# finleygou/GS-MARL

Measured on NVIDIA B200. Metric: agent-steps/sec (graph obs+reward+cost) at 1/2/4/8 B200; % HBM roofline, higher is better.
Workload: dtype f32

## Files before the change

gs_marl_b200/csrc/gsm_kernels.cuh:

```cuda
#pragma once
#include <cuda_runtime.h>
#include <math.h>
#include <stdint.h>

#include "../../include/gsmarl_b200.h"
#include "gsm_host.h"

namespace gsm {

constexpr int kThreads = 128;
__host__ __device__ constexpr unsigned low_mask(int n) { return n >= 32 ? 0xffffffffu : ((1u << (n & 31)) - 1u); }

template <typename T>
struct KParams {
  int64_t n_envs, env_offset;
  int N, L, E, K, W;
  int scenario, action_mode, n_actions, episode_length;
  int share_reward, cost_obstacles, own_goal_always;
  int envs_per_warp;
  T dt, one_minus_damp, cf, km, km_inv, Rs, w_dist, w_goal, goal_tol, poly_r;
  T discrete_u[GSM_MAX_DISCRETE][2];
  const T* size;
  const uint8_t* eflag;
  const T* mass;
  const T* accel;
  const T* max_speed;
  const T* slot_table;
  T* agent_state;
  T* lm_pos;
  int32_t* t;
  const uint8_t* mask;
  int64_t mask_stride;
  int auto_reset;
  uint64_t seed;
  int32_t* episode;
  double ext[4];
  const void* actions;
  T* obs; int32_t* nbr_idx; T* nbr_feat; int32_t* nbr_cnt; uint32_t* adj;
  T* reward; T* cost; uint8_t* done; int32_t* assign;
};

struct SmemLayout {
  size_t off_size, off_agc, off_ag, off_lm, off_new, off_rew, off_slot, off_cmat, off_asg,
      off_stage, off_flag, stage_stride, stage_feat, total;
};
__host__ __device__ inline SmemLayout make_layout(int rb, int N, int L, int E, int K, int epb,
                                                  int groups, int lsa) {
  SmemLayout s;
  size_t o = 0;
  auto take = [&](size_t bytes) { size_t r = o; o += ((bytes + 15) / 16) * 16; return r; };
  s.off_size = take((size_t)E * rb);
  s.off_agc = take((size_t)N * 3 * rb);
  s.off_ag = take((size_t)epb * N * 4 * rb);
  s.off_lm = take((size_t)epb * L * 2 * rb);
  s.off_new = take((size_t)epb * N * 4 * rb);
  s.off_rew = take((size_t)epb * N * rb);
  s.off_slot = take(lsa ? (size_t)epb * N * 2 * rb : 0);
  s.off_cmat = take(lsa ? (size_t)epb * N * N * rb : 0);
  s.off_asg = take((size_t)epb * N * 4);
  s.stage_feat = (((size_t)K * 4 + 15) / 16) * 16;
  s.stage_stride = s.stage_feat + (((size_t)K * GSM_NBR_FEAT_DIM * rb + 15) / 16) * 16;
  s.off_stage = take((size_t)groups * s.stage_stride);
  s.off_flag = take((size_t)E);
  s.total = o;
  return s;
}

__device__ __forceinline__ float r_sqrt(float x) { return sqrtf(x); }
__device__ __forceinline__ double r_sqrt(double x) { return sqrt(x); }
__device__ __forceinline__ float r_exp(float x) { return expf(x); }
__device__ __forceinline__ double r_exp(double x) { return exp(x); }
__device__ __forceinline__ float r_log1p(float x) { return log1pf(x); }
__device__ __forceinline__ double r_log1p(double x) { return log1p(x); }

template <typename T>
__device__ __forceinline__ T softplus(T x) {
  if (x > (T)0) return x + r_log1p(r_exp(-x));
  return r_log1p(r_exp(x));
}

__device__ __forceinline__ float shfl(unsigned m, float v, int src) { return __shfl_sync(m, v, src); }
__device__ __forceinline__ double shfl(unsigned m, double v, int src) { return __shfl_sync(m, v, src); }
__device__ __forceinline__ int shfl(unsigned m, int v, int src) { return __shfl_sync(m, v, src); }

__device__ __forceinline__ float mask_min(unsigned m, float v) {
  unsigned b = __float_as_uint(v);
  unsigned key = (b & 0x80000000u) ? ~b : (b | 0x80000000u);
  unsigned r = __reduce_min_sync(m, key);
  return __uint_as_float((r & 0x80000000u) ? (r & 0x7fffffffu) : ~r);
}
__device__ __forceinline__ double mask_min(unsigned m, double v) {
  unsigned long long b = (unsigned long long)__double_as_longlong(v);
  unsigned long long key = (b >> 63) ? ~b : (b | 0x8000000000000000ull);
  unsigned hi = (unsigned)(key >> 32), lo = (unsigned)key;
  unsigned mhi = __reduce_min_sync(m, hi);
  unsigned mlo = __reduce_min_sync(m, hi == mhi ? lo : 0xffffffffu);
  unsigned long long r = ((unsigned long long)mhi << 32) | mlo;
  r = (r >> 63) ? (r & 0x7fffffffffffffffull) : ~r;
  return __longlong_as_double((long long)r);
}

template <typename T> __device__ __forceinline__ T r_inf();
template <> __device__ __forceinline__ float r_inf<float>() { return __int_as_float(0x7f800000); }
template <> __device__ __forceinline__ double r_inf<double>() {
  return __longlong_as_double(0x7ff0000000000000ll);
}

__device__ __forceinline__ void philox4x32_10(uint32_t c0, uint32_t c1, uint32_t c2, uint32_t c3,
                                              uint32_t k0, uint32_t k1, uint32_t out[4]);
__device__ __forceinline__ double u53(uint32_t hi, uint32_t lo);
static __device__ __noinline__ void spawn_draw_f64(uint64_t g, int ep, int e, uint64_t seed, double ext,
                                            double* x, double* y) {
  uint32_t r[4];
  philox4x32_10((uint32_t)g, (uint32_t)(g >> 32), (uint32_t)ep, (uint32_t)e, (uint32_t)seed,
                (uint32_t)(seed >> 32), r);
  *x = __dadd_rn(-ext, __dmul_rn(2.0 * ext, u53(r[0], r[1])));
  *y = __dadd_rn(-ext, __dmul_rn(2.0 * ext, u53(r[2], r[3])));
}
template <typename T>
__device__ __forceinline__ void spawn_draw(uint64_t g, int ep, int e, uint64_t seed, double ext, T& x, T& y) {
  double dx, dy;
  spawn_draw_f64(g, ep, e, seed, ext, &dx, &dy);
  x = (T)dx; y = (T)dy;
}

template <typename T> struct Prec;
template <> struct Prec<float> { static constexpr bool kCut = true; };
template <> struct Prec<double> { static constexpr bool kCut = false; };
constexpr float kFarCut = 20.0f;

template <int P>
__device__ __forceinline__ void group_copy(void* gdst, const void* ssrc, int bytes, int sub) {
  const uintptr_t ga = (uintptr_t)gdst;
  if (((ga | (uintptr_t)bytes) & 15) == 0) {
    for (int k = sub; k < (bytes >> 4); k += P) ((int4*)gdst)[k] = ((const int4*)ssrc)[k];
  } else if (((ga | (uintptr_t)bytes) & 7) == 0) {
    for (int k = sub; k < (bytes >> 3); k += P) ((int2*)gdst)[k] = ((const int2*)ssrc)[k];
  } else {
    for (int k = sub; k < (bytes >> 2); k += P) ((int*)gdst)[k] = ((const int*)ssrc)[k];
  }
}

template <typename T>
__device__ int lsa_lanes(const T* __restrict__ C, int n, int col, unsigned gm, int base) {
  const T INF = r_inf<T>();
  T u_m = 0, v_m = 0;
  int col4row_m = -1, row4col_m = -1, path_m = -1;
  const bool is_col = col < n;
  for (int cur = 0; cur < n; cur++) {
    T minval = 0, spc = INF;
    int i = cur, nrem = n, sink = -1;
    int pos = n - 1 - col;
    bool inrem = is_col, sr_m = false, sc_m = false;
    for (int iter = 0; iter < n && sink == -1; iter++) {
      if (col == i) sr_m = true;
      const T u_i = shfl(gm, u_m, base + i);
      if (inrem) {
        const T r = minval + C[i * n + col] - u_i - v_m;
        if (r < spc) { path_m = i; spc = r; }
      }
      const T lowest = mask_min(gm, inrem ? spc : INF);
      if (lowest == INF) return -1;
      const bool cand = inrem && spc == lowest;
      const bool ucand = cand && row4col_m == -1;
      const unsigned bu = __ballot_sync(gm, ucand);
      int selpos;
      if (bu) selpos = __reduce_max_sync(gm, ucand ? pos : -1);
      else selpos = __reduce_min_sync(gm, cand ? pos : 0x3fffffff);
      const bool sel = inrem && pos == selpos;
      const int jl = __ffs(__ballot_sync(gm, sel)) - 1;
      minval = lowest;
      const int r4c = shfl(gm, row4col_m, jl);
      if (r4c == -1) sink = jl - base; else i = r4c;
      if (sel) { sc_m = true; inrem = false; }
      nrem--;
      if (inrem && pos == nrem) pos = selpos;
    }
    const T spc_row = shfl(gm, spc, base + (col4row_m >= 0 ? col4row_m : 0));
    if (is_col) {
      if (col == cur) u_m += minval;
      else if (sr_m) u_m += minval - spc_row;
    }
    if (sc_m) v_m -= minval - spc;
    if (sink < 0) return -1;
    int j = sink;
    for (int iter = 0; iter < n; iter++) {
      const int a = shfl(gm, path_m, base + j);
      if (col == j) row4col_m = a;
      const int tprev = shfl(gm, col4row_m, base + a);
      if (col == a) col4row_m = j;
      j = tprev;
      if (a == cur) break;
    }
  }
  return col4row_m;
}

template <typename T, int N>
__device__ __forceinline__ int lsa_seg(const T* __restrict__ C, int off, int base, bool live) {
  constexpr unsigned FULL = 0xffffffffu;
  const T INF = r_inf<T>();
  const bool is_col = live && off < N;
  T u_m = 0, v_m = 0;
  int col4row_m = -1, row4col_m = -1, path_m = -1;
  for (int cur = 0; cur < N; cur++) {
    T minval = 0, spc = INF;
    int i = cur, nrem = N, sink = live ? -1 : 0;
    int rem = N - 1 - off;
    bool inrem = is_col, sr_m = false, sc_m = false;
    for (int iter = 0; iter < N && __any_sync(FULL, sink == -1); iter++) {
      const bool run = sink == -1;
      if (run && off == i) sr_m = true;
      const T u_i = shfl(FULL, u_m, base + i);
      if (run && inrem) {
        const T r = minval + C[i * N + off] - u_i - v_m;
        if (r < spc) { path_m = i; spc = r; }
      }
      const T mine = inrem ? spc : INF;
      T lowest = INF;
#pragma unroll
      for (int k = 0; k < N; k++) {
        const T o = shfl(FULL, mine, base + k);
        lowest = o < lowest ? o : lowest;
      }
      const int rc = off < N ? rem : 0;
      const T spc_of = shfl(FULL, spc, base + rc);
      const int r4c_of = shfl(FULL, row4col_m, base + rc);
      const bool cand = is_col && off < nrem && spc_of == lowest;
      const bool ucand = cand && r4c_of == -1;
      const unsigned bc = (__ballot_sync(FULL, cand) >> base) & low_mask(N);
      const unsigned bu = (__ballot_sync(FULL, ucand) >> base) & low_mask(N);
      const int it_sel = bu ? (31 - __clz(bu)) : (bc ? __ffs(bc) - 1 : 0);
      const int j = shfl(FULL, rem, base + it_sel);
      const int r4c_j = shfl(FULL, row4col_m, base + j);
      const int last = shfl(FULL, rem, base + nrem - 1);
      if (run) {
        minval = lowest;
        if (r4c_j == -1) sink = j; else i = r4c_j;
        if (off == j) { sc_m = true; inrem = false; }
        if (off == it_sel) rem = last;
        nrem--;
      }
    }
    const T spc_row = shfl(FULL, spc, base + (col4row_m >= 0 ? col4row_m : 0));
    if (is_col) {
      if (off == cur) u_m += minval;
      else if (sr_m) u_m += minval - spc_row;
    }
    if (sc_m) v_m -= minval - spc;
    int j = sink;
    bool going = live && sink >= 0;
    for (int iter = 0; iter < N && __any_sync(FULL, going); iter++) {
      const int a = shfl(FULL, path_m, base + j);
      const int tprev = shfl(FULL, col4row_m, base + a);
      if (going) {
        if (off == j) row4col_m = a;
        if (off == a) col4row_m = j;
        j = tprev;
        if (a == cur) going = false;
      }
    }
  }
  return col4row_m;
}

template <typename T, int P, bool CTA_ENV, bool PHYS>
__global__ void __launch_bounds__(kThreads) env_kernel(const __grid_constant__ KParams<T> p) {
  extern __shared__ __align__(16) unsigned char smem[];
  const int N = p.N, L = p.L, E = p.E, K = p.K, W = p.W;
  const bool lsa = p.scenario != GSM_SCN_NAVIGATION;
  const int EPB = CTA_ENV ? 1 : p.envs_per_warp * (kThreads / 32);
  const SmemLayout lay = make_layout((int)sizeof(T), N, L, E, K, EPB, kThreads / P, lsa ? 1 : 0);
  T* s_size = (T*)(smem + lay.off_size);
  T* s_agc = (T*)(smem + lay.off_agc);
  T* s_ag = (T*)(smem + lay.off_ag);
// ... 370 lines not shown
```

gs_marl_b200/csrc/gsm_kernels_wide.cuh:

```cuda
#pragma once
#include "gsm_kernels_spec.cuh"
#include "gsm_bulk.cuh"

namespace gsm {

constexpr int kWideThreads = 128;
__host__ __device__ constexpr int wide_pow2(int v) { int p = 1; while (p < v) p <<= 1; return p; }

template <typename T, int N, int E>
struct WideConsts {
  T size[E];
  T mass[N], mass_inv[N], accel[N], maxsp[N];
  int32_t eflag[E];
};

#ifndef GSM_WIDE_BLOCKS
#define GSM_WIDE_BLOCKS 7
#endif
template <typename T> struct WideMinBlocks { static constexpr int value = sizeof(T) == 4 ? GSM_WIDE_BLOCKS : 1; };

__device__ __forceinline__ float softplus1(float x) {
  float y, l;
  asm("ex2.approx.ftz.f32 %0, %1;" : "=f"(y) : "f"(-fabsf(x) * 1.4426950408889634f));
  asm("lg2.approx.ftz.f32 %0, %1;" : "=f"(l) : "f"(1.0f + y));
  return fmaxf(x, 0.f) + 0.6931471805599453f * l;
}
__device__ __forceinline__ double softplus1(double x) { return fmax(x, 0.0) + r_log1p(r_exp(-fabs(x))); }

__device__ __forceinline__ int keep(int v) { return __shfl_sync(0xffffffffu, v, threadIdx.x & 31); }
__device__ __forceinline__ unsigned keep(unsigned v) { return __shfl_sync(0xffffffffu, v, threadIdx.x & 31); }
__device__ __forceinline__ float keep(float v) { return __shfl_sync(0xffffffffu, v, threadIdx.x & 31); }
__device__ __forceinline__ double keep(double v) { return __shfl_sync(0xffffffffu, v, threadIdx.x & 31); }

__device__ __forceinline__ void sts(unsigned a, unsigned v) { asm volatile("st.shared.u32 [%0], %1;" :: "r"(a), "r"(v) : "memory"); }
__device__ __forceinline__ void sts(unsigned a, int v) { asm volatile("st.shared.u32 [%0], %1;" :: "r"(a), "r"(v) : "memory"); }
__device__ __forceinline__ void sts(unsigned a, float v) { asm volatile("st.shared.f32 [%0], %1;" :: "r"(a), "f"(v) : "memory"); }
__device__ __forceinline__ void sts(unsigned a, double v) { asm volatile("st.shared.f64 [%0], %1;" :: "r"(a), "d"(v) : "memory"); }
__device__ __forceinline__ void sts2(unsigned a, float x, float y) { asm volatile("st.shared.v2.f32 [%0], {%1, %2};" :: "r"(a), "f"(x), "f"(y) : "memory"); }
__device__ __forceinline__ void sts2(unsigned a, double x, double y) { asm volatile("st.shared.v2.f64 [%0], {%1, %2};" :: "r"(a), "d"(x), "d"(y) : "memory"); }
__device__ __forceinline__ void sts4(unsigned a, float x, float y, float z, float w) {
  asm volatile("st.shared.v4.f32 [%0], {%1, %2, %3, %4};" :: "r"(a), "f"(x), "f"(y), "f"(z), "f"(w) : "memory");
}
__device__ __forceinline__ void sts4(unsigned a, double x, double y, double z, double w) { sts2(a, x, y); sts2(a + 16, z, w); }
__device__ __forceinline__ void lds4(unsigned a, float& x, float& y, float& z, float& w) {
  asm volatile("ld.shared.v4.f32 {%0, %1, %2, %3}, [%4];" : "=f"(x), "=f"(y), "=f"(z), "=f"(w) : "r"(a) : "memory");
}
__device__ __forceinline__ void lds4(unsigned a, double& x, double& y, double& z, double& w) {
  asm volatile("ld.shared.v2.f64 {%0, %1}, [%2];" : "=d"(x), "=d"(y) : "r"(a) : "memory");
  asm volatile("ld.shared.v2.f64 {%0, %1}, [%2];" : "=d"(z), "=d"(w) : "r"(a + 16) : "memory");
}
__device__ __forceinline__ float4 lds16(unsigned a) {
  float4 v; asm volatile("ld.shared.v4.f32 {%0, %1, %2, %3}, [%4];" : "=f"(v.x), "=f"(v.y), "=f"(v.z), "=f"(v.w) : "r"(a) : "memory"); return v;
}

template <typename T>
__device__ __forceinline__ T shfl_xor(T v, int m) { return __shfl_xor_sync(0xffffffffu, v, m); }

template <typename T> struct __align__(16) WideEnt { T x, y, vx, vy; };

struct WideSmem {
  unsigned feat, idx, obs, cnt, adj, cost, rew, asg, buf;
  unsigned ent, warp;
};
__host__ __device__ constexpr WideSmem wide_smem_layout(int rb, int N, int E, int K, int EPW) {
  WideSmem w{};
  unsigned o = 0;
  w.feat = o; o += (unsigned)(EPW * N * K * GSM_NBR_FEAT_DIM * rb);
  w.idx = o; o += ((unsigned)(EPW * N * K * 4) + 15u) & ~15u;
  w.obs = o; o += (unsigned)(EPW * N * GSM_OBS_DIM * rb);
  w.cnt = o; o += (unsigned)(EPW * N * 4);
  w.adj = o; o += (unsigned)(EPW * N * 4);
  w.cost = o; o += (unsigned)(EPW * N * rb);
  w.rew = o; o += (unsigned)(EPW * N * rb);
  w.asg = o; o += (unsigned)(EPW * N * 4);
  w.buf = (o + 15u) & ~15u;
  w.ent = 2 * w.buf;
  w.warp = w.ent + (unsigned)(EPW * E * 4 * rb);
  return w;
}
__host__ __device__ constexpr size_t wide_smem_bytes(int rb, int N, int E, int K, int EPW) {
  return (size_t)(kWideThreads / 32) * wide_smem_layout(rb, N, E, K, EPW).warp;
}

template <typename T, int N, int L, int MODE, int KT>
__global__ void __launch_bounds__(kWideThreads, WideMinBlocks<T>::value)
env_wide_kernel(const __grid_constant__ KParams<T> p, const int n_steps,
                const __grid_constant__ StepStrides ss,
                const __grid_constant__ WideConsts<T, N, N + L> wc,
                const __grid_constant__ WideSmem lay_rt) {
  constexpr int E = N + L, M = E - 1, GW = wide_pow2(M), EPW = 32 / GW;
  constexpr bool OBS = MODE == 1;
  constexpr unsigned FULL = 0xffffffffu;
  constexpr int RB = (int)sizeof(T);
  constexpr int RS4 = EPW * N * 4, RST = EPW * N * RB;
  constexpr int PS = (RS4 % 16 == 0 && RST % 16 == 0) ? 16 : 8;
  constexpr int PC4 = RS4 / PS, PCT = RST / PS, NPIECE = 3 * PC4 + 2 * PCT;
  constexpr bool ROLE_OK = NPIECE <= 32;
  static_assert(GW <= 32 && E <= 32, "an env must fit in one warp, adjacency in one word");
  static_assert(L >= N && 2 * N <= GW + 1 && N >= 3, "goal i is landmark i, held by lane N-1+i; lanes 0..2 stage scalars");
  static_assert(RS4 % 8 == 0 && RST % 8 == 0, "per-warp scalar blocks leave in 8- or 16-byte pieces");
  static_assert(EPW * N * M * 4 / 16 <= 64 && EPW * N * GSM_OBS_DIM * RB / 16 <= 64, "idx / obs blocks leave in <= 2 passes");
  typedef Arith<T> A;
  typedef WideEnt<T> Ent;
  typedef float4 V;
  extern __shared__ __align__(128) unsigned char wsm[];
  const int K = KT > 0 ? KT : p.K;
  const WideSmem lay = KT > 0 ? wide_smem_layout((int)sizeof(T), N, N + L, KT > 0 ? KT : 1, 32 / wide_pow2(N + L - 1)) : lay_rt;
  const int lane = keep((int)(threadIdx.x & 31)), warp = threadIdx.x >> 5;
  const int grp = lane / GW, j = lane % GW, shift = grp * GW;
  const int env_w0 = keep((int)(((int64_t)blockIdx.x * (kWideThreads / 32) + warp) * EPW));
  bool active = env_w0 + grp < p.n_envs;
  if (OBS && p.mask != nullptr && active) active = p.mask[(int64_t)(env_w0 + grp) * p.mask_stride] != 0;
  const int env = active ? env_w0 + grp : 0;
  const bool has = M == GW ? true : j < M;
  const bool own = j < N;
  const int ja = own ? j : 0;
  const unsigned act_bits = __ballot_sync(FULL, active);
  const bool bulk = ROLE_OK && act_bits == FULL && ((EPW * N * K * 4) & 15) == 0 &&
      ((((uintptr_t)p.obs | (uintptr_t)p.nbr_idx | (uintptr_t)p.nbr_feat | (uintptr_t)p.nbr_cnt | (uintptr_t)p.adj |
         (uintptr_t)p.assign | (uintptr_t)p.reward | (uintptr_t)p.cost | (uintptr_t)ss.obs | (uintptr_t)ss.nbr_idx |
         (uintptr_t)ss.nbr_feat | (uintptr_t)ss.nbr_cnt | (uintptr_t)ss.adj | (uintptr_t)ss.assign |
         (uintptr_t)ss.reward | (uintptr_t)ss.cost) & 15) == 0);

  constexpr unsigned ES = (unsigned)sizeof(Ent);
  const unsigned sa_w = keep(smem_u32(wsm) + (unsigned)warp * lay.warp);
  const unsigned sa_ent = keep(smem_u32(wsm) + (unsigned)warp * lay.warp + lay.ent + (unsigned)(grp * E) * ES);

  const int e_hi = has ? j + 1 : 0;
  const int fl_o = wc.eflag[e_hi];
  const T size_o = keep(wc.size[e_hi]), type_o = keep((T)(fl_o >> 1));
  const unsigned lfl = keep((unsigned)((has && (wc.eflag[0] & 1) && (fl_o & 1)) ? 1u : 0u) |
                            ((has && (e_hi < N || (p.cost_obstacles && (fl_o >> 1) == GSM_ENT_OBSTACLE))) ? 2u : 0u) |
                            (((has && p.own_goal_always && j >= N - 1 && j < 2 * N - 1) ? (unsigned)(j - (N - 1) + 1) : 0u) << 8));
  const bool cpair = lfl & 1u, colc = lfl & 2u;
  const int goal_i = (int)(lfl >> 8) - 1;

  T mx, my, mvx, mvy;
  {
    const T* a = p.agent_state + ((int64_t)env * N + ja) * 4;
    mx = a[0]; my = a[1]; mvx = a[2]; mvy = a[3];
  }
  if (own) sts4(sa_ent + (unsigned)j * ES, mx, my, mvx, mvy);
  if (has && j + 1 >= N) {
    const T* l = p.lm_pos + ((int64_t)env * L + (j + 1 - N)) * 2;
    sts4(sa_ent + (unsigned)(j + 1) * ES, l[0], l[1], (T)0, (T)0);
  }
  int t_now = p.t[env];
  const bool auto_reset = MODE == 2 && p.auto_reset != 0;
  const T accel_m = keep(wc.accel[ja]), mass_m = keep(wc.mass[ja]), massinv_m = keep(wc.mass_inv[ja]), maxsp_m = keep(wc.maxsp[ja]);

  const unsigned char* b_act = (const unsigned char*)p.actions;
  unsigned char* b_obs = (unsigned char*)p.obs;
  unsigned char* b_idx = (unsigned char*)p.nbr_idx;
  unsigned char* b_feat = (unsigned char*)p.nbr_feat;
  unsigned char* b_done = (unsigned char*)p.done;
  const unsigned wrow0 = (unsigned)env_w0 * N;
  unsigned char* c_role = nullptr;
  int64_t role_stride = ss.nbr_cnt;
  {
    const int q = lane;
    if (q < PC4) c_role = (unsigned char*)p.nbr_cnt + wrow0 * 4u + q * PS;
    else if (q < 2 * PC4) { c_role = (unsigned char*)p.adj + wrow0 * 4u + (q - PC4) * PS; if (RB != 4) role_stride = ss.adj; }
    else if (q < 2 * PC4 + PCT) { c_role = (unsigned char*)p.cost + wrow0 * (unsigned)RB + (q - 2 * PC4) * PS; if (RB != 4) role_stride = ss.cost; }
    else if (q < 2 * PC4 + 2 * PCT) { c_role = (unsigned char*)p.reward + wrow0 * (unsigned)RB + (q - 2 * PC4 - PCT) * PS; if (RB != 4) role_stride = ss.reward; }
    else if (q < NPIECE) { c_role = (unsigned char*)p.assign + wrow0 * 4u + (q - 2 * PC4 - 2 * PCT) * PS; if (RB != 4) role_stride = ss.assign; }
  }
  const bool role_on = lane < NPIECE && (!OBS || lane < 2 * PC4 || lane >= 2 * PC4 + 2 * PCT);
  if (own) {
    sts(sa_w + lay.asg + (unsigned)(grp * N + j) * 4u, j);
    sts(sa_w + lay.buf + lay.asg + (unsigned)(grp * N + j) * 4u, j);
  }

  const bool discrete = p.action_mode == GSM_ACT_DISCRETE;
  const unsigned act_off = keep(discrete ? ((unsigned)env * N + ja) * 4u : ((unsigned)env * N + ja) * 2u * (unsigned)RB);
  const unsigned n_idx = (lay.obs - lay.idx) / 16, n_obs = (lay.cnt - lay.obs) / 16;
  const unsigned off_idx = keep(wrow0 * (unsigned)(K * 4) + (unsigned)lane * 16u), off_obs = keep(wrow0 * (unsigned)(GSM_OBS_DIM * RB) + (unsigned)lane * 16u);
  const unsigned off_done = keep((unsigned)env * N + (unsigned)ja);
  int act_next = 0;
  T actx_next = 0, acty_next = 0;
  if (!OBS) {
    if (discrete) act_next = *(const int32_t*)(b_act + act_off);
    else { actx_next = ((const T*)(b_act + act_off))[0]; acty_next = ((const T*)(b_act + act_off))[1]; }
  }
  __syncwarp();

  T fox = 0, foy = 0;
  bool pro = !OBS;
  int step = 0;
  unsigned sb = sa_w;
  int sb_delta = (int)lay.buf;
  const unsigned o_feat = keep((unsigned)(grp * N * K) * (unsigned)(GSM_NBR_FEAT_DIM * RB));
  const unsigned o_idx = keep(lay.idx + (unsigned)(grp * N * K) * 4u);
  const unsigned o_sc = keep(lay.cnt + (unsigned)(j < 3 ? j : 0) * (unsigned)RS4 + (unsigned)(grp * N) * 4u);
  const unsigned o_obs = keep(lay.obs + (unsigned)grp * (unsigned)(N * GSM_OBS_DIM * RB));
  while (step < n_steps) {
   for (;;) {
    if (!OBS && !pro) {
      T ux = actx_next, uy = acty_next;
      if (discrete) {
        const int a = act_next;
        ux = 0; uy = 0;
        if (a >= 0 && a < p.n_actions) { ux = p.discrete_u[a][0]; uy = p.discrete_u[a][1]; }
      }
      if (step + 1 < n_steps) b_act += ss.actions;
      if (discrete) act_next = *(const int32_t*)(b_act + act_off);
      else { actx_next = ((const T*)(b_act + act_off))[0]; acty_next = ((const T*)(b_act + act_off))[1]; }
      const T fx = accel_m * ux + fox, fy = accel_m * uy + foy;
      T nvx = mvx * p.one_minus_damp, nvy = mvy * p.one_minus_damp;
      nvx = nvx + A::div_const(fx, mass_m, massinv_m) * p.dt;
      nvy = nvy + A::div_const(fy, mass_m, massinv_m) * p.dt;
      if (maxsp_m > (T)0) {
        const T sp = A::sqrt(nvx * nvx + nvy * nvy);
        if (sp > maxsp_m) { nvx = A::div(nvx, sp) * maxsp_m; nvy = A::div(nvy, sp) * maxsp_m; }
      }
      mvx = nvx; mvy = nvy;
      mx = mx + nvx * p.dt; my = my + nvy * p.dt;
      t_now += 1;
      if (own) sts4(sa_ent + (unsigned)j * ES, mx, my, mvx, mvy);
      __syncwarp();
    }
    const bool st_on = !pro;
    const unsigned a_feat = sb + o_feat, a_idx = sb + o_idx, a_sc = sb + o_sc, sobs = sb + o_obs;
    if (st_on && bulk && lane == 0) bulk_wait_read<1>();

    T fcx[N], fcy[N];
    T gxs = 0, gys = 0, gd = 0;
    bool anyc = false;
#pragma unroll
    for (int i = 0; i < N; i++) {
      const int e = e_hi - (j < i ? 1 : 0);
      Ent si, so;
      lds4(sa_ent + (unsigned)i * ES, si.x, si.y, si.vx, si.vy);
      lds4(sa_ent + (unsigned)e * ES, so.x, so.y, so.vx, so.vy);
      const T dx = so.x - si.x, dy = so.y - si.y;
      const T dist = A::sqrt(dx * dx + dy * dy);
      const T dmin = wc.size[i] + size_o;
      const bool nb = (has && dist < p.Rs) || goal_i == i;
      const bool col = colc && dist < dmin;
      const unsigned bits = (__ballot_sync(FULL, nb) >> shift) & low_mask(GW);
      const unsigned cbits = (__ballot_sync(FULL, col) >> shift) & low_mask(GW);
      int cnt = __popc(bits);
      const int rank = __popc(bits & low_mask(j));
      const int pos = nb ? rank : cnt + (j - rank);
      if (has && pos < K && st_on) {
        sts(a_idx + (unsigned)pos * 4u + (unsigned)(i * K * 4), nb ? e : -1);
        const unsigned f = a_feat + (unsigned)pos * (unsigned)(GSM_NBR_FEAT_DIM * RB) + (unsigned)(i * K * GSM_NBR_FEAT_DIM * RB);
        const T z = (T)0;
        if (nb) { sts2(f, dx, dy); sts2(f + 2 * RB, so.vx - si.vx, so.vy - si.vy); sts2(f + 4 * RB, dist, type_o); }
        else { sts2(f, z, z); sts2(f + 2 * RB, z, z); sts2(f + 4 * RB, z, z); }
      }
      if (cnt > K) cnt = K;
      if (st_on && j < 3) {
        const unsigned ebits = (bits & low_mask(i)) | ((bits & ~low_mask(i)) << 1);
        const unsigned ao = (unsigned)(grp * N + i);
        if (RB == 4) {
          const unsigned v = j == 0 ? (unsigned)cnt : (j == 1 ? ebits : __float_as_uint((float)__popc(cbits)));
          if (!OBS || j < 2) sts(a_sc + (unsigned)(i * 4), v);
        } else {
          if (j == 0) sts(sb + lay.cnt + ao * 4u, cnt);
          else if (j == 1) sts(sb + lay.adj + ao * 4u, ebits);
          else if (!OBS) sts(sb + lay.cost + ao * (unsigned)RB, (T)__popc(cbits));
        }
      }
      if (j == N - 1 + i) { gxs = dx; gys = dy; gd = dist; }
      if (!OBS) {
        fcx[i] = 0; fcy[i] = 0;
        if (cpair) {
          const T x = A::div_const(-(dist - dmin), p.km, p.km_inv);
          if (!(Prec<T>::kCut && x < (T)(-kFarCut))) {
            const T pen = softplus1(x) * p.km;
            fcx[i] = A::div(p.cf * (-dx), dist) * pen;
            fcy[i] = A::div(p.cf * (-dy), dist) * pen;
            anyc = true;
          }
        }
      }
    }
    if (!OBS && (pro || step + 1 < n_steps)) {
      fox = 0; foy = 0;
      if (__any_sync(FULL, anyc)) {
#pragma unroll
        for (int m = GW / 2; m >= 1; m >>= 1) {
#pragma unroll
          for (int i = 0; i < N; i++) { fcx[i] = fcx[i] + shfl_xor(fcx[i], m); fcy[i] = fcy[i] + shfl_xor(fcy[i], m); }
        }
#pragma unroll
        for (int i = 0; i < N; i++) if (ja == i) { fox = fcx[i]; foy = fcy[i]; }
      }
    }

    if (st_on) {
      if (own) { sts2(sobs + (unsigned)j * (GSM_OBS_DIM * RB), mvx, mvy); sts2(sobs + (unsigned)j * (GSM_OBS_DIM * RB) + 2 * RB, mx, my); }
      T rs = ((T)0 - p.w_dist * gd) + (gd < p.goal_tol ? p.w_goal : (T)0);
      if (p.share_reward && !OBS) {
        T s = shfl(FULL, rs, shift + N - 1);
#pragma unroll
        for (int k = 1; k < N; k++) s = s + shfl(FULL, rs, shift + N - 1 + k);
        rs = s / (T)N;
      }
      if (j >= N - 1 && j < 2 * N - 1) {
        const unsigned ao = (unsigned)(j - (N - 1));
        sts2(sobs + ao * (GSM_OBS_DIM * RB) + 4 * RB, gxs, gys);
        if (!OBS) sts(sb + lay.rew + ((unsigned)grp * N + ao) * (unsigned)RB, rs);
      }
      if (!OBS && own && active) b_done[off_done] = (uint8_t)(t_now >= p.episode_length);
      if (bulk) {
        fence_async_smem();
        __syncwarp();
        if (lane == 0) {
          asm volatile("cp.async.bulk.global.shared::cta.bulk_group [%0], [%1], %2;"
                       :: "l"(b_feat + wrow0 * (unsigned)(K * GSM_NBR_FEAT_DIM * RB)), "r"(sb), "r"(lay.idx) : "memory");
          bulk_commit();
        }
        V* const g_idx = (V*)(b_idx + off_idx);
        V* const g_obs = (V*)(b_obs + off_obs);
        const unsigned s_idx = sb + lay.idx + (unsigned)lane * 16u, s_obs = sb + lay.obs + (unsigned)lane * 16u;
        if (lane < n_idx) g_idx[0] = lds16(s_idx);
        if (lane + 32 < n_idx) g_idx[32] = lds16(s_idx + 512);
        if (lane < n_obs) g_obs[0] = lds16(s_obs);
        if (lane + 32 < n_obs) g_obs[32] = lds16(s_obs + 512);
        if (role_on) {
          if (PS == 16) *(V*)c_role = lds16(sb + lay.cnt + (unsigned)lane * 16u);
          else {
            float2 v8;
            asm volatile("ld.shared.v2.f32 {%0, %1}, [%2];" : "=f"(v8.x), "=f"(v8.y) : "r"(sb + lay.cnt + (unsigned)lane * 8u) : "memory");
            *(float2*)c_role = v8;
          }
        }
      } else {
        __syncwarp();
        auto copy_words = [&](unsigned char* g, unsigned soff, unsigned bytes) {
          const unsigned wpe = bytes / (4 * EPW);
          for (unsigned q = lane; q < bytes / 4; q += 32)
            if ((act_bits >> ((q / wpe) * GW)) & 1u) {
              unsigned v; asm volatile("ld.shared.u32 %0, [%1];" : "=r"(v) : "r"(sb + soff + q * 4u) : "memory");
              ((uint32_t*)g)[q] = v;
            }
        };
        copy_words(b_feat + wrow0 * (unsigned)(K * GSM_NBR_FEAT_DIM * RB), lay.feat, lay.idx - lay.feat);
        copy_words(b_idx + wrow0 * (unsigned)(K * 4), lay.idx, (unsigned)(EPW * N * K * 4));
        copy_words(b_obs + wrow0 * (unsigned)(GSM_OBS_DIM * RB), lay.obs, lay.cnt - lay.obs);
        copy_words((unsigned char*)p.nbr_cnt + (int64_t)step * ss.nbr_cnt + wrow0 * 4u, lay.cnt, RS4);
        copy_words((unsigned char*)p.adj + (int64_t)step * ss.adj + wrow0 * 4u, lay.adj, RS4);
        copy_words((unsigned char*)p.assign + (int64_t)step * ss.assign + wrow0 * 4u, lay.asg, RS4);
        if (!OBS) {
          copy_words((unsigned char*)p.reward + (int64_t)step * ss.reward + wrow0 * (unsigned)RB, lay.rew, RST);
          copy_words((unsigned char*)p.cost + (int64_t)step * ss.cost + wrow0 * (unsigned)RB, lay.cost, RST);
        }
        __syncwarp();
      }
    }
    if (OBS) break;
    if (pro) { pro = false; continue; }
    b_obs += ss.obs; b_idx += ss.nbr_idx; b_feat += ss.nbr_feat; b_done += ss.done;
    c_role += role_stride;
    sb += sb_delta;
    sb_delta = -sb_delta;
    step++;
    if (step >= n_steps) break;
    if (MODE == 2 && auto_reset && __any_sync(FULL, t_now >= p.episode_length)) break;
   }
   if (OBS) break;
   if (MODE == 2 && auto_reset) {
     const bool fin = t_now >= p.episode_length;
     if (__any_sync(FULL, fin)) {
       __syncwarp();
       if (fin) {
         const uint64_t genv = (uint64_t)(p.env_offset + env);
         const int ep = p.episode[env];
         spawn_draw<T>(genv, ep, ja, p.seed, p.ext[GSM_ENT_AGENT], mx, my);
         mvx = 0; mvy = 0;
         if (own) sts4(sa_ent + (unsigned)j * ES, mx, my, (T)0, (T)0);
         if (has && j + 1 >= N) {
           T lx, ly;
           spawn_draw<T>(genv, ep, j + 1, p.seed, p.ext[wc.eflag[j + 1] >> 1], lx, ly);
           sts4(sa_ent + (unsigned)(j + 1) * ES, lx, ly, (T)0, (T)0);
           if (active) { T* l = p.lm_pos + ((int64_t)env * L + (j + 1 - N)) * 2; l[0] = lx; l[1] = ly; }
         }
         t_now = 0;
       }
       __syncwarp();
       if (fin && j == 0 && active) p.episode[env] += 1;
       __syncwarp();
       pro = step < n_steps;
     }
   }
  }
  if (bulk && lane == 0) bulk_wait_read<0>();

  if (!OBS && active) {
    if (own) {
      T* a = p.agent_state + ((int64_t)env * N + j) * 4;
      st2<T>(a, mx, my); st2<T>(a + 2, mvx, mvy);
    }
    if (j == 0) p.t[env] = t_now;
  }
}

}
```

profiles/sweep_nav3.py:

```python
import argparse
import json
import os
import subprocess
import sys

ROOT = os.path.dirname(os.path.dirname(os.path.abspath(__file__)))


def child(args):
    sys.path.insert(0, ROOT)
    import torch
    from bench_util import time_rollouts
    from gs_marl_b200 import scenarios
    from gs_marl_b200.environment import MultiAgentGraphConstrainEnv, StreamShardedEnv
    N, n_envs, T = args.agents, args.envs, args.T
    cfg = scenarios.load(args.scenario).make_world(N, dtype="f32", episode_length=25)
    dev = torch.device("cuda", 0)
    acts = torch.randint(0, 5, (T, n_envs, N), device=dev, dtype=torch.int32)
    one = MultiAgentGraphConstrainEnv(cfg, n_envs, seed=1)
    one.reset()
    ring = {k: one._alloc(k, (T,)) for k in one.OUTPUTS}
    sh = StreamShardedEnv(cfg, n_envs, n_streams=args.streams, seed=1)
    sh.reset()
    peak = 6546.2
    out = {}
    for name, env in (("s4", sh), ("s1", one)):
        for mode, auto in (("auto", True), ("plain", False)):
            r = time_rollouts(env, cfg, acts, ring, args.K, T, auto, args.ms)
            out[f"{name}_{mode}_us"] = round(r["step_us"], 3)
            out[f"{name}_{mode}_frac"] = round(r["achieved"] / peak, 4)
    torch.cuda.synchronize()
    out["checksum"] = float(ring["nbr_feat"].double().sum().item() + ring["reward"].double().sum().item()
                            + ring["nbr_idx"].double().sum().item() + ring["obs"].double().sum().item())
    print("RESULT " + json.dumps(out), flush=True)


def main():
    ap = argparse.ArgumentParser()
    ap.add_argument("--variants", default="base")
    ap.add_argument("--child", action="store_true")
    ap.add_argument("--scenario", default="navigation")
    ap.add_argument("--agents", type=int, default=3)
    ap.add_argument("--envs", type=int, default=16384)
    ap.add_argument("--T", type=int, default=25)
    ap.add_argument("--K", type=int, default=25)
    ap.add_argument("--streams", type=int, default=4)
    ap.add_argument("--ms", type=float, default=150.0)
    ap.add_argument("--json", default=None)
    args = ap.parse_args()
    if args.child:
        return child(args)
    res = {}
    for v in args.variants.split(","):
        name, *kvs = v.split(":")
        env, streams = dict(os.environ), args.streams
        for kv in kvs:
            k, val = kv.split("=", 1)
            if k == "lib":
                env["GSM_LIB_PATH"] = os.path.join(ROOT, val)
            elif k == "streams":
                streams = int(val)
            else:
                env[k] = val
        cmd = [sys.executable, os.path.abspath(__file__), "--child", "--scenario", args.scenario, "--agents",
               str(args.agents), "--envs", str(args.envs), "--T", str(args.T), "--K", str(args.K), "--streams",
               str(streams), "--ms", str(args.ms)]
        p = subprocess.run(cmd, env=env, capture_output=True, text=True, timeout=600)
        line = [ln for ln in p.stdout.splitlines() if ln.startswith("RESULT ")]
        res[name] = json.loads(line[0][7:]) if line else {"error": (p.stderr or p.stdout)[-400:]}
        print(f"{name:14s} {json.dumps(res[name])}", flush=True)
    if args.json:
        json.dump(res, open(args.json, "w"), indent=1)


if __name__ == "__main__":
    main()
```

Measured before the change: 14.13 billion.

## Prefetch auto-reset spawn draws in wide kernel and plan step runs per warp

For the wide kernel in auto-reset mode with 8-sized entity groups, spawn positions for the next episode are drawn ahead of time into a shared-memory staging area, using an inlined Philox path. Each warp also computes how many steps remain before any of its envs finishes, so the per-step any_sync episode check becomes a precomputed stop bound. At reset, staged positions are copied in from shared memory instead of being drawn inline. Landmark positions and episode counters are written back only when they changed. This costs extra shared memory per env, which may lower occupancy, and adds more control-flow complexity.

```diff
diff --git a/gs_marl_b200/csrc/gsm_kernels.cuh b/gs_marl_b200/csrc/gsm_kernels.cuh
--- a/gs_marl_b200/csrc/gsm_kernels.cuh
+++ b/gs_marl_b200/csrc/gsm_kernels.cuh
@@ -109,18 +109,23 @@
 __device__ __forceinline__ void philox4x32_10(uint32_t c0, uint32_t c1, uint32_t c2, uint32_t c3,
                                               uint32_t k0, uint32_t k1, uint32_t out[4]);
 __device__ __forceinline__ double u53(uint32_t hi, uint32_t lo);
-static __device__ __noinline__ void spawn_draw_f64(uint64_t g, int ep, int e, uint64_t seed, double ext,
-                                            double* x, double* y) {
+__device__ __forceinline__ void spawn_draw_body(uint64_t g, int ep, int e, uint64_t seed, double ext,
+                                                double& x, double& y) {
   uint32_t r[4];
   philox4x32_10((uint32_t)g, (uint32_t)(g >> 32), (uint32_t)ep, (uint32_t)e, (uint32_t)seed,
                 (uint32_t)(seed >> 32), r);
-  *x = __dadd_rn(-ext, __dmul_rn(2.0 * ext, u53(r[0], r[1])));
-  *y = __dadd_rn(-ext, __dmul_rn(2.0 * ext, u53(r[2], r[3])));
-}
-template <typename T>
+  x = __dadd_rn(-ext, __dmul_rn(2.0 * ext, u53(r[0], r[1])));
+  y = __dadd_rn(-ext, __dmul_rn(2.0 * ext, u53(r[2], r[3])));
+}
+static __device__ __noinline__ void spawn_draw_f64(uint64_t g, int ep, int e, uint64_t seed, double ext,
+                                            double* x, double* y) {
+  spawn_draw_body(g, ep, e, seed, ext, *x, *y);
+}
+template <typename T, bool INL = false>
 __device__ __forceinline__ void spawn_draw(uint64_t g, int ep, int e, uint64_t seed, double ext, T& x, T& y) {
   double dx, dy;
-  spawn_draw_f64(g, ep, e, seed, ext, &dx, &dy);
+  if (INL) spawn_draw_body(g, ep, e, seed, ext, dx, dy);
+  else spawn_draw_f64(g, ep, e, seed, ext, &dx, &dy);
   x = (T)dx; y = (T)dy;
 }
 
diff --git a/gs_marl_b200/csrc/gsm_kernels_wide.cuh b/gs_marl_b200/csrc/gsm_kernels_wide.cuh
--- a/gs_marl_b200/csrc/gsm_kernels_wide.cuh
+++ b/gs_marl_b200/csrc/gsm_kernels_wide.cuh
@@ -14,6 +14,9 @@
   int32_t eflag[E];
 };
 
+#ifndef GSM_WIDE_DIAG
+#define GSM_WIDE_DIAG 0
+#endif
 #ifndef GSM_WIDE_BLOCKS
 #define GSM_WIDE_BLOCKS 7
 #endif
@@ -49,6 +52,15 @@
   asm volatile("ld.shared.v2.f64 {%0, %1}, [%2];" : "=d"(x), "=d"(y) : "r"(a) : "memory");
   asm volatile("ld.shared.v2.f64 {%0, %1}, [%2];" : "=d"(z), "=d"(w) : "r"(a + 16) : "memory");
 }
+__device__ __forceinline__ void lds2(unsigned a, float& x, float& y) {
+  asm volatile("ld.shared.v2.f32 {%0, %1}, [%2];" : "=f"(x), "=f"(y) : "r"(a) : "memory");
+}
+__device__ __forceinline__ void lds2(unsigned a, double& x, double& y) {
+  asm volatile("ld.shared.v2.f64 {%0, %1}, [%2];" : "=d"(x), "=d"(y) : "r"(a) : "memory");
+}
+__device__ __forceinline__ int lds_i(unsigned a) {
+  int v; asm volatile("ld.shared.u32 %0, [%1];" : "=r"(v) : "r"(a) : "memory"); return v;
+}
 __device__ __forceinline__ float4 lds16(unsigned a) {
   float4 v; asm volatile("ld.shared.v4.f32 {%0, %1, %2, %3}, [%4];" : "=f"(v.x), "=f"(v.y), "=f"(v.z), "=f"(v.w) : "r"(a) : "memory"); return v;
 }
@@ -57,12 +69,16 @@
 __device__ __forceinline__ T shfl_xor(T v, int m) { return __shfl_xor_sync(0xffffffffu, v, m); }
 
 template <typename T> struct __align__(16) WideEnt { T x, y, vx, vy; };
-
+__host__ __device__ constexpr unsigned wide_env_bytes(int rb, int E, bool next) {
+  return next ? (((unsigned)(E * 4 * rb + E * 2 * rb + 16) + 15u) & ~15u) : (unsigned)(E * 4 * rb);
+}
+
+__host__ __device__ constexpr bool wide_prefetch(int E) { return wide_pow2(E - 1) == 8; }
 struct WideSmem {
   unsigned feat, idx, obs, cnt, adj, cost, rew, asg, buf;
   unsigned ent, warp;
 };
-__host__ __device__ constexpr WideSmem wide_smem_layout(int rb, int N, int E, int K, int EPW) {
+__host__ __device__ constexpr WideSmem wide_smem_layout(int rb, int N, int E, int K, int EPW, bool next) {
   WideSmem w{};
   unsigned o = 0;
   w.feat = o; o += (unsigned)(EPW * N * K * GSM_NBR_FEAT_DIM * rb);
@@ -75,11 +91,11 @@
   w.asg = o; o += (unsigned)(EPW * N * 4);
   w.buf = (o + 15u) & ~15u;
   w.ent = 2 * w.buf;
-  w.warp = w.ent + (unsigned)(EPW * E * 4 * rb);
+  w.warp = w.ent + (unsigned)(EPW * wide_env_bytes(rb, E, next));
   return w;
 }
-__host__ __device__ constexpr size_t wide_smem_bytes(int rb, int N, int E, int K, int EPW) {
-  return (size_t)(kWideThreads / 32) * wide_smem_layout(rb, N, E, K, EPW).warp;
+__host__ __device__ constexpr size_t wide_smem_bytes(int rb, int N, int E, int K, int EPW, bool next) {
+  return (size_t)(kWideThreads / 32) * wide_smem_layout(rb, N, E, K, EPW, next).warp;
 }
 
 template <typename T, int N, int L, int MODE, int KT>
@@ -90,6 +106,7 @@
                 const __grid_constant__ WideSmem lay_rt) {
   constexpr int E = N + L, M = E - 1, GW = wide_pow2(M), EPW = 32 / GW;
   constexpr bool OBS = MODE == 1;
+  constexpr bool PF = MODE == 2 && wide_prefetch(E);
   constexpr unsigned FULL = 0xffffffffu;
   constexpr int RB = (int)sizeof(T);
   constexpr int RS4 = EPW * N * 4, RST = EPW * N * RB;
@@ -105,7 +122,7 @@
   typedef float4 V;
   extern __shared__ __align__(128) unsigned char wsm[];
   const int K = KT > 0 ? KT : p.K;
-  const WideSmem lay = KT > 0 ? wide_smem_layout((int)sizeof(T), N, N + L, KT > 0 ? KT : 1, 32 / wide_pow2(N + L - 1)) : lay_rt;
+  const WideSmem lay = KT > 0 ? wide_smem_layout((int)sizeof(T), N, N + L, KT > 0 ? KT : 1, 32 / wide_pow2(N + L - 1), PF) : lay_rt;
   const int lane = keep((int)(threadIdx.x & 31)), warp = threadIdx.x >> 5;
   const int grp = lane / GW, j = lane % GW, shift = grp * GW;
   const int env_w0 = keep((int)(((int64_t)blockIdx.x * (kWideThreads / 32) + warp) * EPW));
@@ -124,7 +141,9 @@
 
   constexpr unsigned ES = (unsigned)sizeof(Ent);
   const unsigned sa_w = keep(smem_u32(wsm) + (unsigned)warp * lay.warp);
-  const unsigned sa_ent = keep(smem_u32(wsm) + (unsigned)warp * lay.warp + lay.ent + (unsigned)(grp * E) * ES);
+  const unsigned sa_ent = keep(smem_u32(wsm) + (unsigned)warp * lay.warp + lay.ent + (unsigned)grp * wide_env_bytes(RB, E, PF));
+  const unsigned sa_next = sa_ent + (unsigned)E * ES;
+  const unsigned sa_ep = sa_next + (unsigned)(E * 2 * RB);
 
   const int e_hi = has ? j + 1 : 0;
   const int fl_o = wc.eflag[e_hi];
@@ -135,18 +154,25 @@
   const bool cpair = lfl & 1u, colc = lfl & 2u;
   const int goal_i = (int)(lfl >> 8) - 1;
 
-  T mx, my, mvx, mvy;
-  {
+  const bool auto_reset = MODE == 2 && p.auto_reset != 0;
+  const bool pf = PF && auto_reset;
+  T mx = 0, my = 0, mvx = 0, mvy = 0;
+  if (!PF || active) {
     const T* a = p.agent_state + ((int64_t)env * N + ja) * 4;
     mx = a[0]; my = a[1]; mvx = a[2]; mvy = a[3];
   }
   if (own) sts4(sa_ent + (unsigned)j * ES, mx, my, mvx, mvy);
   if (has && j + 1 >= N) {
-    const T* l = p.lm_pos + ((int64_t)env * L + (j + 1 - N)) * 2;
-    sts4(sa_ent + (unsigned)(j + 1) * ES, l[0], l[1], (T)0, (T)0);
-  }
-  int t_now = p.t[env];
-  const bool auto_reset = MODE == 2 && p.auto_reset != 0;
+    T lx = 0, ly = 0;
+    if (!PF || active) { const T* l = p.lm_pos + ((int64_t)env * L + (j + 1 - N)) * 2; lx = l[0]; ly = l[1]; }
+    sts4(sa_ent + (unsigned)(j + 1) * ES, lx, ly, (T)0, (T)0);
+  }
+  int t_now = 0, ep = 0;
+  if (!PF || active) {
+    t_now = p.t[env];
+    if (pf && !GSM_WIDE_DIAG) ep = p.episode[env];
+  }
+  if (pf && j == 0) { sts(sa_ep, ep); sts(sa_ep + 4, ep); sts(sa_ep + 8, env); }
   const T accel_m = keep(wc.accel[ja]), mass_m = keep(wc.mass[ja]), massinv_m = keep(wc.mass_inv[ja]), maxsp_m = keep(wc.maxsp[ja]);
 
   const unsigned char* b_act = (const unsigned char*)p.actions;
@@ -193,6 +219,15 @@
   const unsigned o_idx = keep(lay.idx + (unsigned)(grp * N * K) * 4u);
   const unsigned o_sc = keep(lay.cnt + (unsigned)(j < 3 ? j : 0) * (unsigned)RS4 + (unsigned)(grp * N) * 4u);
   const unsigned o_obs = keep(lay.obs + (unsigned)grp * (unsigned)(N * GSM_OBS_DIM * RB));
+  int stop = n_steps;
+  auto plan = [&]() {
+    const unsigned rem = !active ? 0xffffffffu : t_now >= p.episode_length ? 1u : (unsigned)(p.episode_length - t_now);
+    const unsigned run = __reduce_min_sync(FULL, rem), left = (unsigned)(n_steps - step);
+    stop = step + (int)(run < left ? run : left);
+    return run <= left;
+  };
+  bool draw = pf && plan();
+  if (draw) stop = step + 1;
   while (step < n_steps) {
    for (;;) {
     if (!OBS && !pro) {
@@ -357,11 +392,56 @@
     sb += sb_delta;
     sb_delta = -sb_delta;
     step++;
-    if (step >= n_steps) break;
-    if (MODE == 2 && auto_reset && __any_sync(FULL, t_now >= p.episode_length)) break;
+    if (step >= (PF ? stop : n_steps)) break;
+    if (MODE == 2 && !PF && auto_reset && __any_sync(FULL, t_now >= p.episode_length)) break;
    }
    if (OBS) break;
-   if (MODE == 2 && auto_reset) {
+   if (PF && auto_reset) {
+   if (draw && active) {
+     const uint64_t genv = (uint64_t)(p.env_offset + lds_i(sa_ep + 8));
+     const int ep = lds_i(sa_ep);
+     T x, y;
+     if (own) {
+#if GSM_WIDE_DIAG
+       x = (T)(0.25 * j); y = (T)(-0.25 * j);
+#else
+       spawn_draw<T, true>(genv, ep, j, p.seed, p.ext[GSM_ENT_AGENT], x, y);
+#endif
+       sts2(sa_next + (unsigned)(j * 2 * RB), x, y);
+     }
+     if (has && j + 1 >= N) {
+#if GSM_WIDE_DIAG
+       x = (T)(0.25 * (j + 1)); y = (T)(-0.25 * (j + 1));
+#else
+       spawn_draw<T, true>(genv, ep, j + 1, p.seed, p.ext[wc.eflag[j + 1] >> 1], x, y);
+#endif
+       sts2(sa_next + (unsigned)((j + 1) * 2 * RB), x, y);
+     }
+   }
+     draw = false;
+     const bool fin = active && t_now >= p.episode_length;
+     if (__any_sync(FULL, fin)) {
+       __syncwarp();
+       if (fin) {
+         lds2(sa_next + (unsigned)(ja * 2 * RB), mx, my);
+         mvx = 0; mvy = 0;
+         if (own) sts4(sa_ent + (unsigned)j * ES, mx, my, (T)0, (T)0);
+         if (has && j + 1 >= N) {
+           T x, y;
+           lds2(sa_next + (unsigned)((j + 1) * 2 * RB), x, y);
+           sts4(sa_ent + (unsigned)(j + 1) * ES, x, y, (T)0, (T)0);
+         }
+         t_now = 0;
+         if (j == 0) sts(sa_ep, lds_i(sa_ep) + 1);
+       }
+       __syncwarp();
+       pro = step < n_steps;
+       draw = __any_sync(FULL, fin && p.episode_length <= n_steps - step);
+     }
+     plan();
+     if (draw) stop = step + 1;
+   }
+   if (MODE == 2 && !PF && auto_reset) {
      const bool fin = t_now >= p.episode_length;
      if (__any_sync(FULL, fin)) {
        __syncwarp();
@@ -389,12 +469,21 @@
   if (bulk && lane == 0) bulk_wait_read<0>();
 
   if (!OBS && active) {
+    const int64_t env_s = pf ? lds_i(sa_ep + 8) : env;
     if (own) {
-      T* a = p.agent_state + ((int64_t)env * N + j) * 4;
+      T* a = p.agent_state + (env_s * N + j) * 4;
       st2<T>(a, mx, my); st2<T>(a + 2, mvx, mvy);
     }
-    if (j == 0) p.t[env] = t_now;
-  }
-}
-
-}
+    if (j == 0) p.t[env_s] = t_now;
+    if (pf && lds_i(sa_ep) != lds_i(sa_ep + 4)) {
+      if (has && j + 1 >= N) {
+        T x, y;
+        lds2(sa_ent + (unsigned)(j + 1) * ES, x, y);
+        st2<T>(p.lm_pos + (env_s * L + (j + 1 - N)) * 2, x, y);
+      }
+      if (j == 0 && !GSM_WIDE_DIAG) p.episode[env_s] = lds_i(sa_ep);
+    }
+  }
+}
+
+}
diff --git a/profiles/sweep_nav3.py b/profiles/sweep_nav3.py
--- a/profiles/sweep_nav3.py
+++ b/profiles/sweep_nav3.py
@@ -14,7 +14,7 @@
     from gs_marl_b200 import scenarios
     from gs_marl_b200.environment import MultiAgentGraphConstrainEnv, StreamShardedEnv
     N, n_envs, T = args.agents, args.envs, args.T
-    cfg = scenarios.load(args.scenario).make_world(N, dtype="f32", episode_length=25)
+    cfg = scenarios.load(args.scenario).make_world(N, dtype="f32", episode_length=args.episode_length)
     dev = torch.device("cuda", 0)
     acts = torch.randint(0, 5, (T, n_envs, N), device=dev, dtype=torch.int32)
     one = MultiAgentGraphConstrainEnv(cfg, n_envs, seed=1)
@@ -45,6 +45,7 @@
     ap.add_argument("--T", type=int, default=25)
     ap.add_argument("--K", type=int, default=25)
     ap.add_argument("--streams", type=int, default=4)
+    ap.add_argument("--episode-length", type=int, default=25)
     ap.add_argument("--ms", type=float, default=150.0)
     ap.add_argument("--json", default=None)
     args = ap.parse_args()
@@ -64,7 +65,7 @@
                 env[k] = val
         cmd = [sys.executable, os.path.abspath(__file__), "--child", "--scenario", args.scenario, "--agents",
                str(args.agents), "--envs", str(args.envs), "--T", str(args.T), "--K", str(args.K), "--streams",
-               str(streams), "--ms", str(args.ms)]
+               str(streams), "--ms", str(args.ms), "--episode-length", str(args.episode_length)]
         p = subprocess.run(cmd, env=env, capture_output=True, text=True, timeout=600)
         line = [ln for ln in p.stdout.splitlines() if ln.startswith("RESULT ")]
         res[name] = json.loads(line[0][7:]) if line else {"error": (p.stderr or p.stdout)[-400:]}
```

Measured after the change: 14.49 billion (median of 6 runs). 2.5% higher.

## Branch-free neighbor stores and force terms, precomputed episode segment ends in wide kernel

Applied to the files above, without the earlier changes.

For the step/reward mode the inner neighbor loop now uses predicated shared stores and selects instead of divergent branches, and always computes the collision force term before masking it. The per-step warp vote on episode end is replaced by a precomputed segment stop found with a warp min-reduce over remaining episode steps. Reset spawning is restructured to loop over entities with an inlined Philox draw. Inactive lanes skip global loads. This trades extra unconditional arithmetic (divisions, softplus) for fewer divergent branches and fewer votes per step.

```diff
diff --git a/gs_marl_b200/csrc/gsm_kernels.cuh b/gs_marl_b200/csrc/gsm_kernels.cuh
--- a/gs_marl_b200/csrc/gsm_kernels.cuh
+++ b/gs_marl_b200/csrc/gsm_kernels.cuh
@@ -109,13 +109,17 @@
 __device__ __forceinline__ void philox4x32_10(uint32_t c0, uint32_t c1, uint32_t c2, uint32_t c3,
                                               uint32_t k0, uint32_t k1, uint32_t out[4]);
 __device__ __forceinline__ double u53(uint32_t hi, uint32_t lo);
-static __device__ __noinline__ void spawn_draw_f64(uint64_t g, int ep, int e, uint64_t seed, double ext,
-                                            double* x, double* y) {
+__device__ __forceinline__ void spawn_draw_inline(uint64_t g, int ep, int e, uint64_t seed, double ext,
+                                                  double& x, double& y) {
   uint32_t r[4];
   philox4x32_10((uint32_t)g, (uint32_t)(g >> 32), (uint32_t)ep, (uint32_t)e, (uint32_t)seed,
                 (uint32_t)(seed >> 32), r);
-  *x = __dadd_rn(-ext, __dmul_rn(2.0 * ext, u53(r[0], r[1])));
-  *y = __dadd_rn(-ext, __dmul_rn(2.0 * ext, u53(r[2], r[3])));
+  x = __dadd_rn(-ext, __dmul_rn(2.0 * ext, u53(r[0], r[1])));
+  y = __dadd_rn(-ext, __dmul_rn(2.0 * ext, u53(r[2], r[3])));
+}
+static __device__ __noinline__ void spawn_draw_f64(uint64_t g, int ep, int e, uint64_t seed, double ext,
+                                            double* x, double* y) {
+  spawn_draw_inline(g, ep, e, seed, ext, *x, *y);
 }
 template <typename T>
 __device__ __forceinline__ void spawn_draw(uint64_t g, int ep, int e, uint64_t seed, double ext, T& x, T& y) {
diff --git a/gs_marl_b200/csrc/gsm_kernels_wide.cuh b/gs_marl_b200/csrc/gsm_kernels_wide.cuh
--- a/gs_marl_b200/csrc/gsm_kernels_wide.cuh
+++ b/gs_marl_b200/csrc/gsm_kernels_wide.cuh
@@ -49,6 +49,24 @@
   asm volatile("ld.shared.v2.f64 {%0, %1}, [%2];" : "=d"(x), "=d"(y) : "r"(a) : "memory");
   asm volatile("ld.shared.v2.f64 {%0, %1}, [%2];" : "=d"(z), "=d"(w) : "r"(a + 16) : "memory");
 }
+__device__ __forceinline__ void sts_if(bool on, unsigned a, unsigned v) {
+  asm volatile("{ .reg .pred q; setp.ne.u32 q, %2, 0; @q st.shared.u32 [%0], %1; }" :: "r"(a), "r"(v), "r"((unsigned)on) : "memory");
+}
+__device__ __forceinline__ void sts2_if(bool on, unsigned a, float x, float y) {
+  asm volatile("{ .reg .pred q; setp.ne.u32 q, %3, 0; @q st.shared.v2.f32 [%0], {%1, %2}; }" :: "r"(a), "f"(x), "f"(y), "r"((unsigned)on) : "memory");
+}
+__device__ __forceinline__ void sts2_if(bool on, unsigned a, double x, double y) {
+  asm volatile("{ .reg .pred q; setp.ne.u32 q, %3, 0; @q st.shared.v2.f64 [%0], {%1, %2}; }" :: "r"(a), "d"(x), "d"(y), "r"((unsigned)on) : "memory");
+}
+__device__ __forceinline__ unsigned selp(bool c, unsigned a, unsigned b) {
+  unsigned r;
+  asm("{ .reg .pred q; setp.ne.u32 q, %3, 0; selp.b32 %0, %1, %2, q; }" : "=r"(r) : "r"(a), "r"(b), "r"((unsigned)c));
+  return r;
+}
+__device__ __forceinline__ float div_eager(float a, float b) {
+  float r; asm volatile("div.approx.f32 %0, %1, %2;" : "=f"(r) : "f"(a), "f"(b)); return r;
+}
+__device__ __forceinline__ double div_eager(double a, double b) { return a / b; }
 __device__ __forceinline__ float4 lds16(unsigned a) {
   float4 v; asm volatile("ld.shared.v4.f32 {%0, %1, %2, %3}, [%4];" : "=f"(v.x), "=f"(v.y), "=f"(v.z), "=f"(v.w) : "r"(a) : "memory"); return v;
 }
@@ -90,6 +108,7 @@
                 const __grid_constant__ WideSmem lay_rt) {
   constexpr int E = N + L, M = E - 1, GW = wide_pow2(M), EPW = 32 / GW;
   constexpr bool OBS = MODE == 1;
+  constexpr bool BF = MODE == 2;
   constexpr unsigned FULL = 0xffffffffu;
   constexpr int RB = (int)sizeof(T);
   constexpr int RS4 = EPW * N * 4, RST = EPW * N * RB;
@@ -135,17 +154,18 @@
   const bool cpair = lfl & 1u, colc = lfl & 2u;
   const int goal_i = (int)(lfl >> 8) - 1;
 
-  T mx, my, mvx, mvy;
-  {
+  T mx = 0, my = 0, mvx = 0, mvy = 0;
+  if (active) {
     const T* a = p.agent_state + ((int64_t)env * N + ja) * 4;
     mx = a[0]; my = a[1]; mvx = a[2]; mvy = a[3];
   }
   if (own) sts4(sa_ent + (unsigned)j * ES, mx, my, mvx, mvy);
   if (has && j + 1 >= N) {
-    const T* l = p.lm_pos + ((int64_t)env * L + (j + 1 - N)) * 2;
-    sts4(sa_ent + (unsigned)(j + 1) * ES, l[0], l[1], (T)0, (T)0);
-  }
-  int t_now = p.t[env];
+    T lx = 0, ly = 0;
+    if (active) { const T* l = p.lm_pos + ((int64_t)env * L + (j + 1 - N)) * 2; lx = l[0]; ly = l[1]; }
+    sts4(sa_ent + (unsigned)(j + 1) * ES, lx, ly, (T)0, (T)0);
+  }
+  int t_now = active ? p.t[env] : 0;
   const bool auto_reset = MODE == 2 && p.auto_reset != 0;
   const T accel_m = keep(wc.accel[ja]), mass_m = keep(wc.mass[ja]), massinv_m = keep(wc.mass_inv[ja]), maxsp_m = keep(wc.maxsp[ja]);
 
@@ -193,6 +213,15 @@
   const unsigned o_idx = keep(lay.idx + (unsigned)(grp * N * K) * 4u);
   const unsigned o_sc = keep(lay.cnt + (unsigned)(j < 3 ? j : 0) * (unsigned)RS4 + (unsigned)(grp * N) * 4u);
   const unsigned o_obs = keep(lay.obs + (unsigned)grp * (unsigned)(N * GSM_OBS_DIM * RB));
+  const auto segment_end = [&]() {
+    int s = n_steps;
+    if (MODE == 2 && auto_reset) {
+      const int left = __reduce_min_sync(FULL, active ? p.episode_length - t_now : INT_MAX);
+      s = step + max(1, min(left, n_steps - step));
+    }
+    return s;
+  };
+  int stop = segment_end();
   while (step < n_steps) {
    for (;;) {
     if (!OBS && !pro) {
@@ -242,7 +271,15 @@
       int cnt = __popc(bits);
       const int rank = __popc(bits & low_mask(j));
       const int pos = nb ? rank : cnt + (j - rank);
-      if (has && pos < K && st_on) {
+      if (BF) {
+        const bool row_on = st_on && has && (KT >= M || pos < K);
+        sts_if(row_on, a_idx + (unsigned)pos * 4u + (unsigned)(i * K * 4), (unsigned)(nb ? e : -1));
+        const unsigned f = a_feat + (unsigned)pos * (unsigned)(GSM_NBR_FEAT_DIM * RB) + (unsigned)(i * K * GSM_NBR_FEAT_DIM * RB);
+        const T z = (T)0;
+        sts2_if(row_on, f, nb ? dx : z, nb ? dy : z);
+        sts2_if(row_on, f + 2 * RB, nb ? so.vx - si.vx : z, nb ? so.vy - si.vy : z);
+        sts2_if(row_on, f + 4 * RB, nb ? dist : z, nb ? type_o : z);
+      } else if (has && pos < K && st_on) {
         sts(a_idx + (unsigned)pos * 4u + (unsigned)(i * K * 4), nb ? e : -1);
         const unsigned f = a_feat + (unsigned)pos * (unsigned)(GSM_NBR_FEAT_DIM * RB) + (unsigned)(i * K * GSM_NBR_FEAT_DIM * RB);
         const T z = (T)0;
@@ -250,8 +287,11 @@
         else { sts2(f, z, z); sts2(f + 2 * RB, z, z); sts2(f + 4 * RB, z, z); }
       }
       if (cnt > K) cnt = K;
-      if (st_on && j < 3) {
-        const unsigned ebits = (bits & low_mask(i)) | ((bits & ~low_mask(i)) << 1);
+      const unsigned ebits = (bits & low_mask(i)) | ((bits & ~low_mask(i)) << 1);
+      if (BF && RB == 4) {
+        const unsigned v = selp(j == 0, (unsigned)cnt, selp(j == 1, ebits, __float_as_uint((float)__popc(cbits))));
+        sts_if(st_on && j < 3, a_sc + (unsigned)(i * 4), v);
+      } else if (st_on && j < 3) {
         const unsigned ao = (unsigned)(grp * N + i);
         if (RB == 4) {
           const unsigned v = j == 0 ? (unsigned)cnt : (j == 1 ? ebits : __float_as_uint((float)__popc(cbits)));
@@ -263,7 +303,15 @@
         }
       }
       if (j == N - 1 + i) { gxs = dx; gys = dy; gd = dist; }
-      if (!OBS) {
+      if (BF) {
+        const T x = A::div_const(-(dist - dmin), p.km, p.km_inv);
+        const bool term = cpair && !(Prec<T>::kCut && x < (T)(-kFarCut));
+        const T pen = softplus1(x) * p.km;
+        const T qx = div_eager(p.cf * (-dx), dist), qy = div_eager(p.cf * (-dy), dist);
+        fcx[i] = term ? qx * pen : (T)0;
+        fcy[i] = term ? qy * pen : (T)0;
+        anyc = anyc || term;
+      } else if (!OBS) {
         fcx[i] = 0; fcy[i] = 0;
         if (cpair) {
           const T x = A::div_const(-(dist - dmin), p.km, p.km_inv);
@@ -357,32 +405,34 @@
     sb += sb_delta;
     sb_delta = -sb_delta;
     step++;
-    if (step >= n_steps) break;
-    if (MODE == 2 && auto_reset && __any_sync(FULL, t_now >= p.episode_length)) break;
+    if (step >= stop) break;
    }
    if (OBS) break;
    if (MODE == 2 && auto_reset) {
-     const bool fin = t_now >= p.episode_length;
+     const bool fin = active && t_now >= p.episode_length;
      if (__any_sync(FULL, fin)) {
        __syncwarp();
+       int ep = 0;
        if (fin) {
          const uint64_t genv = (uint64_t)(p.env_offset + env);
-         const int ep = p.episode[env];
-         spawn_draw<T>(genv, ep, ja, p.seed, p.ext[GSM_ENT_AGENT], mx, my);
+         ep = p.episode[env];
+#pragma unroll 1
+         for (int e = j; e < E; e += GW) {
+           double dx, dy;
+           spawn_draw_inline(genv, ep, e, p.seed, p.ext[wc.eflag[e] >> 1], dx, dy);
+           const T x = (T)dx, y = (T)dy;
+           sts4(sa_ent + (unsigned)e * ES, x, y, (T)0, (T)0);
+           if (e < N) { mx = x; my = y; }
+           else { T* l = p.lm_pos + ((int64_t)env * L + (e - N)) * 2; l[0] = x; l[1] = y; }
+         }
          mvx = 0; mvy = 0;
-         if (own) sts4(sa_ent + (unsigned)j * ES, mx, my, (T)0, (T)0);
-         if (has && j + 1 >= N) {
-           T lx, ly;
-           spawn_draw<T>(genv, ep, j + 1, p.seed, p.ext[wc.eflag[j + 1] >> 1], lx, ly);
-           sts4(sa_ent + (unsigned)(j + 1) * ES, lx, ly, (T)0, (T)0);
-           if (active) { T* l = p.lm_pos + ((int64_t)env * L + (j + 1 - N)) * 2; l[0] = lx; l[1] = ly; }
-         }
          t_now = 0;
        }
        __syncwarp();
-       if (fin && j == 0 && active) p.episode[env] += 1;
+       if (fin && j == 0) p.episode[env] = ep + 1;
        __syncwarp();
        pro = step < n_steps;
+       stop = segment_end();
      }
    }
   }
```

Result: faster. 14.10 billion before, 16.23 billion after (median of 6 runs) (+15.1%).
